# dominikh/jello

Hardware: AMD Instinct MI355X
Metric: Mpixels/sec fine-raster + paths/sec, 100k-path 4096^2 scene (higher is better)
Workload: dtype f32

## Files before the change

### jello_amd/csrc/kernels_tile.hip

```cpp
#include <algorithm>

#include "kcommon.h"

using namespace jk;
using namespace jd;

namespace {

struct Bb4 { float v[4]; };

JD void bbox_intersect(const float* a, const float* b, float* o) {
    float r0 = fmax_(a[0], b[0]), r1 = fmax_(a[1], b[1]), r2 = fmin_(a[2], b[2]), r3 = fmin_(a[3], b[3]);
    o[0] = r0; o[1] = r1; o[2] = r2; o[3] = r3;
}

template <int PASS>
__global__ __launch_bounds__(JL_WG) void k_binning(const JlConfig* __restrict__ cfg, Buf<JlDrawMonoid> draw_monoids, Buf<JlPathBbox> path_bbox_buf,
                                                   Buf<Bb4> clip_bbox_buf, Buf<Bb4> intersected_bbox, JlBump* __restrict__ bump,
                                                   Buf<uint32_t> bin_data, Buf<JlBinHeader> bin_header, uint32_t* __restrict__ wg_tot) {
    __shared__ uint32_t sh_bitmaps[8][JL_N_TILE];
    __shared__ uint32_t sh[8];
    const float SX = 0.00390625f, SY = 0.00390625f;
    uint32_t lid = threadIdx.x;
    uint32_t gid = blockIdx.x * JL_WG + lid;
// ... 139 lines not shown
    const MonoidK<2> sums = block_reduce_monoid<2>(part, sh);
    __syncthreads();
    const uint32_t wg_off = sums.v[0], total = sums.v[1];
    if (blockIdx.x >= write_blocks) {
        tile_zero_part(cfg, total, tiles, blockIdx.x - write_blocks, gridDim.x - write_blocks);
        return;
    }
    if (blockIdx.x == 0u && threadIdx.x == 0u) bump->tile = total;
    uint32_t wg_first = blockIdx.x * JL_WG;
    uint32_t drawobj_ix = wg_first + threadIdx.x;
    uint32_t wg_cnt;
    uint32_t my_sub = block_excl_scan_u32(counts[drawobj_ix], sh, &wg_cnt);
    uint32_t offset = wg_off;
    if (offset + wg_cnt > cfg->tiles_size) {
        offset = 0u;
        if (threadIdx.x == JL_WG - 1u) atomicOr(&bump->failed, (uint32_t)JL_STAGE_TILE_ALLOC);
    }
    if (drawobj_ix < cfg->layout.n_drawobj && paths.ok(drawobj_ix)) paths.p[drawobj_ix].tiles = offset + my_sub;
}
JD void tile_zero_part(const JlConfig* __restrict__ cfg, uint32_t total, Buf<JlTile> tiles, uint32_t block, uint32_t blocks) {
    const uint32_t n = umin_(umin_(total, cfg->tiles_size), tiles.n);
    uint4* p = (uint4*)tiles.p;
    const uint32_t n2 = n >> 1;
    for (uint32_t i = block * JL_WG + threadIdx.x; i < n2; i += blocks * JL_WG) p[i] = make_uint4(0u, 0u, 0u, 0u);
    if ((n & 1u) != 0u && block == 0u && threadIdx.x == 0u) {
        JlTile z;
        z.backdrop = 0;
        z.segment_count_or_ix = 0u;
        tiles.p[n - 1u] = z;
    }
}

__global__ void k_path_count_setup(const JlBump* __restrict__ bump, JlIndirectCount* __restrict__ ind) {
    if (bump->failed != 0u) ind->x = 0u; else ind->x = (bump->lines + (JL_WG - 1u)) / JL_WG;
    ind->y = 1u;
    ind->z = 1u;
}
__global__ void k_path_tiling_setup(const JlBump* __restrict__ bump, JlIndirectCount* __restrict__ ind, Buf<uint32_t> ptcl) {
    if (bump->failed != 0u) {
        ind->x = 0u;
        ptcl.wr(0u, ~0u);
    } else {
        ind->x = (bump->seg_counts + (JL_WG - 1u)) / JL_WG;
    }
    ind->y = 1u;
    ind->z = 1u;
}

#define ONE_MINUS_ULP 0.99999994f
#define ROBUST_EPSILON 2e-7f
#define TILE_SCALE 0.0625f

struct LineSetup {
    bool valid;
    bool is_down, is_positive_slope;
    float a, b, x0, y0, x_sign, s0y;
    uint32_t imin, imax;
    int32_t ymin, ymax, delta;
    int32_t bbox[4];
    int32_t stride;
    uint32_t tiles;
};

JD LineSetup line_setup(const JlLineSoup& line, const Buf<JlPath>& paths) {
    LineSetup r;
    r.valid = false;
    V2 lp0 = v2(line.p0[0], line.p0[1]), lp1 = v2(line.p1[0], line.p1[1]);
    bool is_down = lp1.y >= lp0.y;
    V2 xy0 = is_down ? lp0 : lp1;
    V2 xy1 = is_down ? lp1 : lp0;
    V2 s0 = xy0 * TILE_SCALE;
    V2 s1 = xy1 * TILE_SCALE;
    uint32_t count_x = cell_span(s0.x, s1.x) - 1u;
    uint32_t count = count_x + cell_span(s0.y, s1.y);
    float dx = abs_(s1.x - s0.x);
    float dy = s1.y - s0.y;
    if (dx + dy == 0.0f) return r;
    if (dy == 0.0f && floor_(s0.y) == s0.y) return r;
    float idxdy = 1.0f / (dx + dy);
    float a = dx * idxdy;
    bool is_positive_slope = s1.x >= s0.x;
    float x_sign = is_positive_slope ? 1.0f : -1.0f;
    float xt0 = floor_(s0.x * x_sign);
    float c = s0.x * x_sign - xt0;
    float y0 = floor_(s0.y);
    float ytop = (s0.y == s1.y) ? ceil_(s0.y) : (y0 + 1.0f);
    float b = fmin_((dy * c + dx * (ytop - s0.y)) * idxdy, ONE_MINUS_ULP);
    float robust_err = floor_(a * ((float)count - 1.0f) + b) - (float)count_x;
    if (robust_err != 0.0f) a -= ROBUST_EPSILON * sign_(robust_err);
    float x0 = xt0 * x_sign + (is_positive_slope ? 0.0f : -1.0f);

    JlPath path = paths.rd(line.path_ix);
    int32_t bbox[4] = {(int32_t)path.bbox[0], (int32_t)path.bbox[1], (int32_t)path.bbox[2], (int32_t)path.bbox[3]};
    float xmin = fmin_(s0.x, s1.x);
    int32_t stride = bbox[2] - bbox[0];
    if (s0.y >= (float)bbox[3] || s1.y <= (float)bbox[1] || xmin >= (float)bbox[2] || stride == 0) return r;
    uint32_t imin = 0u;
    if (s0.y < (float)bbox[1]) {
        float iminf = round_(((float)bbox[1] - y0 + b - a) / (1.0f - a)) - 1.0f;
        if (y0 + iminf - floor_(a * iminf + b) < (float)bbox[1]) iminf += 1.0f;
        imin = to_u32(iminf);
    }
    uint32_t imax = count;
    if (s1.y > (float)bbox[3]) {
        float imaxf = round_(((float)bbox[3] - y0 + b - a) / (1.0f - a)) - 1.0f;
        if (y0 + imaxf - floor_(a * imaxf + b) < (float)bbox[3]) imaxf += 1.0f;
        imax = to_u32(imaxf);
    }
    int32_t delta = is_down ? -1 : 1;
    int32_t ymin = 0, ymax = 0;
    if (fmax_(s0.x, s1.x) <= (float)bbox[0]) {
        ymin = to_i32(ceil_(s0.y));
        ymax = to_i32(ceil_(s1.y));
        imax = imin;
    } else {
        float fudge = is_positive_slope ? 0.0f : 1.0f;
        if (xmin < (float)bbox[0]) {
            float f = round_((x_sign * ((float)bbox[0] - x0) - b + fudge) / a);
            if ((x0 + x_sign * floor_(a * f + b) < (float)bbox[0]) == is_positive_slope) f += 1.0f;
            int32_t ynext = to_i32(y0 + f - floor_(a * f + b) + 1.0f);
            if (is_positive_slope) {
                if (to_u32(f) > imin) {
                    ymin = to_i32(y0 + ((y0 == s0.y) ? 0.0f : 1.0f));
                    ymax = ynext;
                    imin = to_u32(f);
                }
            } else {
                if (to_u32(f) < imax) {
                    ymin = ynext;
                    ymax = to_i32(ceil_(s1.y));
                    imax = to_u32(f);
                }
            }
        }
        if (fmax_(s0.x, s1.x) > (float)bbox[2]) {
            float f = round_((x_sign * ((float)bbox[2] - x0) - b + fudge) / a);
            if ((x0 + x_sign * floor_(a * f + b) < (float)bbox[2]) == is_positive_slope) f += 1.0f;
            if (is_positive_slope) imax = umin_(imax, to_u32(f)); else imin = umax_(imin, to_u32(f));
        }
    }
    imax = umax_(imin, imax);
    ymin = imax_(ymin, bbox[1]);
    ymax = imin_(ymax, bbox[3]);
    r.valid = true;
    r.is_down = is_down; r.is_positive_slope = is_positive_slope;
    r.a = a; r.b = b; r.x0 = x0; r.y0 = y0; r.x_sign = x_sign; r.s0y = s0.y;
    r.imin = imin; r.imax = imax; r.ymin = ymin; r.ymax = ymax; r.delta = delta;
    r.bbox[0] = bbox[0]; r.bbox[1] = bbox[1]; r.bbox[2] = bbox[2]; r.bbox[3] = bbox[3];
    r.stride = stride;
    r.tiles = path.tiles;
    return r;
}

__global__ __launch_bounds__(JL_WG) void k_pc_count(const JlBump* __restrict__ bump, const JlIndirectCount* __restrict__ ind, Buf<JlLineSoup> lines,
                                                    Buf<JlPath> paths, uint32_t* __restrict__ counts, uint32_t counts_n,
                                                    uint32_t* __restrict__ zero, uint32_t zero_n, uint32_t* __restrict__ ptotal, uint32_t ptotal_n,
                                                    unsigned long long* __restrict__ bd_ctr,
                                                    JlIndirectCount* __restrict__ setup_out) {
    for (uint32_t i = blockIdx.x * JL_WG + threadIdx.x; i < zero_n; i += gridDim.x * JL_WG) zero[i] = 0u;
    if (blockIdx.x == 0u && threadIdx.x == 0u) *bd_ctr = 0ull;
    uint32_t n_lines = umin_(bump->lines, counts_n);
    uint32_t ind_x;
    if (setup_out) {
        ind_x = bump->failed != 0u ? 0u : (bump->lines + (JL_WG - 1u)) / JL_WG;
        if (blockIdx.x == 0u && threadIdx.x == 0u) { setup_out->x = ind_x; setup_out->y = 1u; setup_out->z = 1u; }
    } else {
        ind_x = ind->x;
    }
    uint32_t n_threads = umin_(ind_x * JL_WG, counts_n);
    const uint32_t lane = lane_id();
    for (uint32_t g0 = blockIdx.x * JL_WG + (threadIdx.x & ~63u); g0 < n_lines; g0 += gridDim.x * JL_WG) {
        const uint32_t gid = g0 + lane;
        uint32_t c = 0u, pix = 0xffffffffu;
        if (gid < n_lines && gid < n_threads && lines.ok(gid)) {
            pix = lines.p[gid].path_ix;
            LineSetup s = line_setup(lines.p[gid], paths);
            if (s.valid) c = s.imax - s.imin;
        }
        if (gid < n_lines) counts[gid] = c;
        const uint32_t incl = wave_incl_scan_u32(c);
        const uint32_t prev = lane_prev(pix, ~pix);
        const uint64_t heads = __builtin_amdgcn_ballot_w64(lane == 0u || pix != prev);
        const uint32_t leader = 63u - (uint32_t)__builtin_clzll(heads & ((2ull << lane) - 1ull));
        const uint32_t lead_incl = (uint32_t)__shfl((int)incl, (int)leader, 64), lead_c = (uint32_t)__shfl((int)c, (int)leader, 64);
        const bool last_of_run = lane == 63u || ((heads >> (lane + 1u)) & 1ull) != 0ull;
        const uint32_t run_sum = incl - (lead_incl - lead_c);
        if (last_of_run && run_sum != 0u && pix < ptotal_n) atomicAdd(&ptotal[pix], run_sum);
    }
}
JD void path_range(uint32_t P, const uint32_t* __restrict__ pstart, const uint32_t* __restrict__ pend, const uint32_t*, const uint32_t*,
                   uint32_t& ps, uint32_t& pe) {
    ps = pstart[P];
    pe = pend[P];
}

#ifndef PC_BIG_PATH
#define PC_BIG_PATH 64u
#endif
JD bool npe_big(uint32_t n) { return n > PC_BIG_PATH; }

#define PC_LONG_LINE 32u
struct EmitCtx {
    const JlConfig* cfg;
    const JlBump* bump;
    Buf<JlTile> tile;
    Buf<JlSegmentCount> seg_counts;
    uint2* tile_of;
    uint32_t* keys;
    uint32_t* kbig;
    uint32_t tile_of_n;
};
JD bool pc_key_is_big(uint32_t key) { return key != 0xffffffffu && (key >> 31) != 0u; }
JD void emit_backdrop_row(const EmitCtx& c, const LineSetup& s, int32_t y) {
    uint32_t base = (uint32_t)((int32_t)s.tiles + (y - s.bbox[1]) * s.stride);
    if (c.tile.ok(base)) atomicAdd(&c.tile.p[base].backdrop, s.delta);
}
template <bool DEFER>
JD void emit_crossing(const EmitCtx& c, const LineSetup& s, uint32_t i, uint32_t gid, uint32_t seg_base, bool big, uint32_t& want_t,
                      uint32_t& want_ix) {
    want_t = 0u;
    want_ix = 0xffffffffu;
    float last_z = floor_(s.a * ((float)i - 1.0f) + s.b);
    float zf = s.a * (float)i + s.b;
    float z = floor_(zf);
    int32_t y = to_i32(s.y0 + (float)i - z);
    int32_t x = to_i32(s.x0 + s.x_sign * z);
    int32_t base = (int32_t)s.tiles + (y - s.bbox[1]) * s.stride - s.bbox[0];
    bool top_edge = (i == 0u) ? (s.y0 == s.s0y) : (last_z == z);
    if (top_edge && x + 1 < s.bbox[2]) {
        int32_t x_bump = imax_(x + 1, s.bbox[0]);
        uint32_t t = (uint32_t)(base + x_bump);
        if (c.tile.ok(t)) atomicAdd(&c.tile.p[t].backdrop, s.delta);
    }
    uint32_t t = (uint32_t)(base + x);
    uint32_t seg_ix = seg_base + i - s.imin;
    if (seg_ix < c.cfg->seg_counts_size && c.seg_counts.ok(seg_ix)) {
        JlSegmentCount sc;
        sc.line_ix = gid;
        sc.counts = i;
        c.seg_counts.p[seg_ix] = sc;
        if (seg_ix < c.tile_of_n) {
            c.keys[seg_ix] = c.tile.ok(t) ? (t | (big ? 0x80000000u : 0u)) : 0xffffffffu;
            if (big) {
                if (DEFER) {
                    want_t = t;
                    want_ix = seg_ix;
                } else {
                    uint32_t arrival = 0u;
                    if (c.tile.ok(t)) arrival = atomicAdd(&c.tile.p[t].segment_count_or_ix, 1u);
                    c.tile_of[seg_ix] = make_uint2(t, arrival);
                }
            }
        }
    }
}

__global__ __launch_bounds__(JL_WG) void k_pc_emit(const JlConfig* __restrict__ cfg, const JlBump* __restrict__ bump,
                                                   const JlIndirectCount* __restrict__ ind, Buf<JlLineSoup> lines, Buf<JlPath> paths, Buf<JlTile> tile,
                                                   Buf<JlSegmentCount> seg_counts, const uint32_t* __restrict__ seg_bases, uint32_t bases_n,
                                                   uint2* __restrict__ tile_of, uint32_t* __restrict__ keys, uint32_t* __restrict__ kbig,
                                                   uint32_t tile_of_n, uint32_t* __restrict__ pfirst, uint32_t* __restrict__ plast,
                                                   const uint32_t* __restrict__ ptotal, uint32_t n_paths, uint32_t* __restrict__ gate) {
    EmitCtx c;
    c.cfg = cfg; c.bump = bump; c.tile = tile; c.seg_counts = seg_counts; c.tile_of = tile_of; c.keys = keys; c.kbig = kbig;
    c.tile_of_n = tile_of_n;
    const uint32_t n_lines = umin_(umin_(bump->lines, bases_n), ind->x * JL_WG);
    const uint32_t lane = lane_id();
    for (uint32_t g0 = blockIdx.x * JL_WG + (threadIdx.x & ~63u); g0 < n_lines; g0 += gridDim.x * JL_WG) {
        const uint32_t gid = g0 + lane;
        LineSetup s;
        s.valid = false;
        uint32_t P = 0xffffffffu;
        uint32_t edgeP = 0xffffffffu;
        if (lane == 0u && gid > 0u && gid - 1u < n_lines && lines.ok(gid - 1u)) edgeP = lines.p[gid - 1u].path_ix;
        if (lane == 63u && gid + 1u < n_lines && lines.ok(gid + 1u)) edgeP = lines.p[gid + 1u].path_ix;
        if (gid < n_lines && lines.ok(gid)) {
            P = lines.p[gid].path_ix;
            s = line_setup(lines.p[gid], paths);
        }
        bool big = true;
        uint32_t seg_base = 0u;
        if (gid < n_lines) seg_base = seg_bases[gid];
        if (s.valid) {
            if (P < n_paths) big = ptotal[P] > PC_BIG_PATH;
        } else {
            s.imin = 0u; s.imax = 0u; s.ymin = 0; s.ymax = 0;
        }
        {
            uint32_t prevP = lane_prev(P, 0u), nextP = lane_next(P, 0u);
            if (lane == 0u) prevP = edgeP;
            if (lane == 63u) nextP = edgeP;
            if (gid < n_lines && P < n_paths) {
                if (P != prevP) pfirst[P] = seg_base;
                if (P != nextP) plast[P] = seg_base + (s.valid ? s.imax - s.imin : 0u);
            }
        }
        if (__builtin_amdgcn_ballot_w64(s.valid && big && s.imax > s.imin) != 0ull && lane == 0u) {
            const uint32_t want = bump->tile;
            if (__hip_atomic_load(gate, __ATOMIC_RELAXED, __HIP_MEMORY_SCOPE_AGENT) < want) atomicMax(gate, want);
        }
        const bool is_long = s.valid && (s.imax - s.imin > PC_LONG_LINE || s.ymax - s.ymin > (int32_t)PC_LONG_LINE);
        const bool per_lane = s.valid && !is_long;
        if (per_lane)
            for (int32_t y = s.ymin; y < s.ymax; y++) emit_backdrop_row(c, s, y);
        uint32_t dummy_t, dummy_ix;
        if (__builtin_amdgcn_ballot_w64(per_lane && big) == 0ull) {
            if (per_lane)
                for (uint32_t i = s.imin; i < s.imax; i++) emit_crossing<false>(c, s, i, gid, seg_base, big, dummy_t, dummy_ix);
        } else {
            const uint32_t trip = per_lane ? s.imax - s.imin : 0u;
            const uint32_t max_trip = (uint32_t)__builtin_amdgcn_readlane((int)wave_incl_max_u32(trip), 63);
            for (uint32_t r = 0u; r < max_trip; r++) {
                uint32_t t = 0u, ix = 0xffffffffu;
                if (r < trip) emit_crossing<true>(c, s, s.imin + r, gid, seg_base, big, t, ix);
                const bool want = ix != 0xffffffffu && c.tile.ok(t);
                const uint32_t key = want ? t : 0xffffffffu - lane;
                const uint32_t prev = (uint32_t)__shfl_up((int)key, 1, 64);
                const bool head = lane == 0u || key != prev;
                const uint64_t heads = __builtin_amdgcn_ballot_w64(head);
                const uint32_t leader = 63u - (uint32_t)__builtin_clzll(heads & ((2ull << lane) - 1ull));
                const uint64_t later = leader == 63u ? 0ull : heads >> (leader + 1u);
                const uint32_t run = later == 0ull ? 64u - leader : (uint32_t)__builtin_ctzll(later) + 1u;
                uint32_t first = 0u;
                if (want && lane == leader) first = atomicAdd(&c.tile.p[t].segment_count_or_ix, run);
                first = (uint32_t)__shfl((int)first, (int)leader, 64);
                if (ix != 0xffffffffu) c.tile_of[ix] = make_uint2(t, want ? first + (lane - leader) : 0u);
            }
        }
        uint64_t m = __builtin_amdgcn_ballot_w64(is_long);
        while (m != 0ull) {
            const uint32_t src = (uint32_t)__builtin_ctzll(m);
            m &= m - 1ull;
            LineSetup t;
            t.valid = true; t.is_down = false; t.is_positive_slope = false;
            t.a = read_lane(s.a, src); t.b = read_lane(s.b, src); t.x0 = read_lane(s.x0, src); t.y0 = read_lane(s.y0, src);
            t.x_sign = read_lane(s.x_sign, src); t.s0y = read_lane(s.s0y, src);
            t.imin = read_lane(s.imin, src); t.imax = read_lane(s.imax, src);
            t.ymin = read_lane(s.ymin, src); t.ymax = read_lane(s.ymax, src); t.delta = read_lane(s.delta, src);
            t.bbox[0] = read_lane(s.bbox[0], src); t.bbox[1] = read_lane(s.bbox[1], src); t.bbox[2] = read_lane(s.bbox[2], src); t.bbox[3] = read_lane(s.bbox[3], src);
            t.stride = read_lane(s.stride, src); t.tiles = read_lane(s.tiles, src);
            const uint32_t t_gid = g0 + src, t_seg_base = read_lane(seg_base, src);
            const bool t_big = read_lane(big ? 1u : 0u, src) != 0u;
            for (int32_t y = t.ymin + (int32_t)lane; y < t.ymax; y += 64) emit_backdrop_row(c, t, y);
            for (uint32_t i = t.imin + lane; i < t.imax; i += 64u) emit_crossing<false>(c, t, i, t_gid, t_seg_base, t_big, dummy_t, dummy_ix);
        }
    }
}

#ifndef PCR_K
#define PCR_K 16u
#endif
struct PcScatterArgs {
    const uint2* tile_of;
    const uint32_t* list_base;
    uint32_t tiles_cap;
    uint32_t* list;
    const uint32_t* kbig;
    uint32_t* gate;
    uint32_t* dense;
    uint32_t dense_cap, blocks;
};
JD void pc_scatter_part(const JlConfig* __restrict__ cfg, const JlBump* __restrict__ bump, Buf<JlTile> tile,
                        const uint2* __restrict__ tile_of, uint32_t n_cap, const uint32_t* __restrict__ list_base,
                        uint32_t tiles_cap, uint32_t* __restrict__ list, const uint32_t* __restrict__ kbig,
                        uint32_t* __restrict__ gate, uint32_t* __restrict__ dense, uint32_t dense_cap, uint32_t block, uint32_t blocks);
__global__ __launch_bounds__(JL_WG) void k_pc_rank_small(const JlConfig* __restrict__ cfg, const JlBump* __restrict__ bump, Buf<JlTile> tile,
                                                         const uint32_t* __restrict__ keys, uint32_t n_cap, const uint32_t* __restrict__ pfirst,
                                                         const uint32_t* __restrict__ plast, const uint32_t* __restrict__ counts,
                                                         const uint32_t* __restrict__ seg_bases, uint32_t n_paths,
                                                         Buf<JlSegmentCount> seg_counts, PcScatterArgs sc, uint32_t* __restrict__ ptotal_zero,
                                                         uint32_t ptotal_words) {
    for (uint32_t i = blockIdx.x * JL_WG + threadIdx.x; i < ptotal_words; i += gridDim.x * JL_WG) ptotal_zero[i] = 0u;
    const uint32_t rank_blocks = gridDim.x - sc.blocks;
    if (blockIdx.x >= rank_blocks) {
        pc_scatter_part(cfg, bump, tile, sc.tile_of, n_cap, sc.list_base, sc.tiles_cap, sc.list, sc.kbig, sc.gate, sc.dense, sc.dense_cap,
                        blockIdx.x - rank_blocks, sc.blocks);
        return;
    }
    const uint32_t n = umin_(umin_(bump->seg_counts, cfg->seg_counts_size), n_cap);
    const uint32_t lane = lane_id();
    const uint32_t waves = (rank_blocks * JL_WG) >> 6;
    const uint32_t wave_ix = (blockIdx.x * JL_WG + threadIdx.x) >> 6;
    const uint32_t n_tasks = (n_paths + PCR_K - 1u) / PCR_K;
    auto load_ranges = [&](uint32_t task, uint32_t& ps, uint32_t& pe) {
        ps = 0u; pe = 0u;
        const uint32_t P = task * PCR_K + lane;
        if (task < n_tasks && lane < PCR_K && P < n_paths) path_range(P, pfirst, plast, counts, seg_bases, ps, pe);
    };
    uint32_t t_ps = 0u, t_pe = 0u;
    uint64_t todo = 0ull;
    uint32_t task = wave_ix;
    uint32_t r_ps, r_pe;
    load_ranges(task, r_ps, r_pe);
    bool task_loaded = false;
    auto advance = [&](uint32_t& cs, uint32_t& ce) -> bool {
        for (;;) {
            if (todo != 0ull) {
                const uint32_t a = (uint32_t)__builtin_ctzll(todo);
                todo &= todo - 1ull;
                cs = (uint32_t)__builtin_amdgcn_readlane((int)t_ps, (int)a);
                ce = (uint32_t)__builtin_amdgcn_readlane((int)t_pe, (int)a);
                while (todo != 0ull) {
                    const uint32_t b2 = (uint32_t)__builtin_ctzll(todo);
                    const uint32_t nps = (uint32_t)__builtin_amdgcn_readlane((int)t_ps, (int)b2);
                    const uint32_t npe = (uint32_t)__builtin_amdgcn_readlane((int)t_pe, (int)b2);
                    if (nps != ce || npe - cs > 64u) break;
                    ce = npe;
                    todo &= todo - 1ull;
                }
                return true;
            }
            if (task_loaded) task += waves;
            if (task >= n_tasks) return false;
            task_loaded = true;
            const uint32_t ps = r_ps, pe_all = r_pe;
            load_ranges(task + waves, r_ps, r_pe);
            t_ps = ps;
            t_pe = umin_(pe_all, n);
            todo = __builtin_amdgcn_ballot_w64(lane < PCR_K && t_pe > ps && !npe_big(pe_all - ps));
        }
    };
    auto fetch = [&](uint32_t cs, uint32_t ce, uint32_t& key, uint32_t& cw) {
        key = 0xffffffffu; cw = 0u;
        const uint32_t k = cs + lane;
        if (k < ce) {
            key = keys[k];
            if (seg_counts.ok(k)) cw = seg_counts.p[k].counts;
        }
    };
    uint32_t c_s = 0u, c_e = 0u, key1 = 0xffffffffu, cw1 = 0u;
    bool have = advance(c_s, c_e);
    if (have) fetch(c_s, c_e, key1, cw1);
    while (have) {
        const uint32_t cs = c_s, ce = c_e;
        const uint32_t my_key = key1, my_cw = cw1;
        have = advance(c_s, c_e);
        if (have) fetch(c_s, c_e, key1, cw1);
        const uint32_t k = cs + lane;
        const bool valid = k < ce;
        const uint32_t my_t = valid ? my_key : 0xffffffffu;
        const bool mine = valid && my_t != 0xffffffffu;
        uint32_t before = 0u, after = 0u;
        uint64_t rem = __builtin_amdgcn_ballot_w64(mine);
        uint32_t grp_lo = 0u, grp_hi = 0u;
        while (rem != 0ull) {
            const uint32_t t = (uint32_t)__builtin_amdgcn_readlane((int)my_t, (int)__builtin_ctzll(rem));
            const bool eq = my_t == t;
            const uint64_t m = __builtin_amdgcn_ballot_w64(eq);
            grp_lo = eq ? (uint32_t)m : grp_lo;
            grp_hi = eq ? (uint32_t)(m >> 32) : grp_hi;
            rem &= ~m;
        }
        if (mine) {
            before = __builtin_amdgcn_mbcnt_hi(grp_hi, __builtin_amdgcn_mbcnt_lo(grp_lo, 0u));
            after = (uint32_t)__builtin_popcount(grp_lo) + (uint32_t)__builtin_popcount(grp_hi) - 1u - before;
        }
        if (mine && seg_counts.ok(k)) {
            seg_counts.p[k].counts = my_cw | (before << 16);
            if (after == 0u && tile.ok(my_t)) tile.p[my_t].segment_count_or_ix = before + 1u;
        }
    }
}

#define PC_DENSE_TILE 16u
#define PC_DENSE_LDS 1024u
JD void pc_scatter_part(const JlConfig* __restrict__ cfg, const JlBump* __restrict__ bump, Buf<JlTile> tile,
                        const uint2* __restrict__ tile_of, uint32_t n_cap, const uint32_t* __restrict__ list_base,
                        uint32_t tiles_cap, uint32_t* __restrict__ list, const uint32_t* __restrict__ kbig,
                        uint32_t* __restrict__ gate, uint32_t* __restrict__ dense, uint32_t dense_cap, uint32_t block, uint32_t blocks) {
    if (*gate == 0u) return;
    uint32_t n = umin_(umin_(bump->seg_counts, cfg->seg_counts_size), n_cap);
    const uint32_t lane = lane_id();
    for (uint32_t k0 = block * JL_WG + (threadIdx.x & ~63u); k0 < n; k0 += blocks * JL_WG) {
        const uint32_t k = k0 + lane;
        bool first_of_dense = false;
        uint32_t t = 0u;
        if (k < n && pc_key_is_big(kbig[k])) {
            uint2 ta = tile_of[k];
            if (ta.x < tiles_cap && tile.ok(ta.x)) {
                uint32_t pos = list_base[ta.x] + ta.y;
                if (pos < n_cap) list[pos] = k;
                t = ta.x;
                first_of_dense = ta.y == 0u && tile.p[t].segment_count_or_ix > PC_DENSE_TILE;
            }
        }
        const uint64_t m = __builtin_amdgcn_ballot_w64(first_of_dense);
        if (m != 0ull) {
            uint32_t at = 0u;
            if (lane == 0u) at = atomicAdd(&gate[1], (uint32_t)__builtin_popcountll(m));
            at = uni(at) + __builtin_amdgcn_mbcnt_hi((uint32_t)(m >> 32), __builtin_amdgcn_mbcnt_lo((uint32_t)m, 0u));
            if (first_of_dense && at < dense_cap) dense[at] = t;
        }
    }
}
__global__ __launch_bounds__(JL_WG) void k_pc_rank(const JlConfig* __restrict__ cfg, const JlBump* __restrict__ bump, Buf<JlTile> tile,
                                                   const uint2* __restrict__ tile_of, uint32_t n_cap, const uint32_t* __restrict__ list_base,
                                                   uint32_t tiles_cap, const uint32_t* __restrict__ list, Buf<JlSegmentCount> seg_counts,
                                                   const uint32_t* __restrict__ kbig, const uint32_t* __restrict__ gate,
                                                   const uint32_t* __restrict__ dense, uint32_t dense_cap) {
    __shared__ uint32_t sh_list[JL_WG / 64][PC_DENSE_LDS];
    if (*gate == 0u) return;
    uint32_t n = umin_(umin_(bump->seg_counts, cfg->seg_counts_size), n_cap);
    for (uint32_t k = blockIdx.x * JL_WG + threadIdx.x; k < n; k += gridDim.x * JL_WG) {
        if (!pc_key_is_big(kbig[k])) continue;
        uint32_t t = tile_of[k].x;
        if (t >= tiles_cap || !tile.ok(t) || !seg_counts.ok(k)) continue;
        uint32_t cnt = tile.p[t].segment_count_or_ix;
        if (cnt > PC_DENSE_TILE) continue;
        uint32_t base = list_base[t];
        uint32_t rank = 0u;
        for (uint32_t j = 0; j < cnt; j++) {
            uint32_t pos = base + j;
            if (pos < n_cap && list[pos] < k) rank++;
        }
        seg_counts.p[k].counts |= rank << 16;
    }
    const uint32_t lane = lane_id(), wv = threadIdx.x >> 6;
    uint32_t* my_list = sh_list[wv];
    const uint32_t n_dense = umin_(gate[1], dense_cap);
    const uint32_t waves = (gridDim.x * JL_WG) >> 6;
    for (uint32_t d = uni((blockIdx.x * JL_WG + threadIdx.x) >> 6); d < n_dense; d += waves) {
        const uint32_t t = uni(dense[d]);
        if (t >= tiles_cap || !tile.ok(t)) continue;
        const uint32_t base = uni(list_base[t]);
        uint32_t m = uni(tile.p[t].segment_count_or_ix);
        if (base >= n_cap) continue;
        m = umin_(m, n_cap - base);
        for (uint32_t o0 = 0u; o0 < m; o0 += PC_DENSE_LDS) {
            const uint32_t on = umin_(m - o0, PC_DENSE_LDS);
            wave_sync();
            for (uint32_t i = lane; i < ((on + 3u) & ~3u); i += 64u) my_list[i] = i < on ? list[base + o0 + i] : 0xffffffffu;
            wave_sync();
            for (uint32_t j = lane; j < m; j += 64u) {
                const uint32_t e = list[base + j];
                uint32_t r = 0u;
                for (uint32_t i = 0u; i < on; i += 4u) {
                    const uint4 q = *(const uint4*)&my_list[i];
                    r += (q.x < e ? 1u : 0u) + (q.y < e ? 1u : 0u) + (q.z < e ? 1u : 0u) + (q.w < e ? 1u : 0u);
                }
                if (seg_counts.ok(e)) seg_counts.p[e].counts += r << 16;
// ... 155 lines not shown
        bool is_positive_slope = s1.x >= s0.x;
        float x_sign = is_positive_slope ? 1.0f : -1.0f;
        float xt0 = floor_(s0.x * x_sign);
        float c = s0.x * x_sign - xt0;
        float y0i = floor_(s0.y);
        float ytop = (s0.y == s1.y) ? ceil_(s0.y) : (y0i + 1.0f);
        float b = fmin_((dy * c + dx * (ytop - s0.y)) * idxdy, ONE_MINUS_ULP);
        float robust_err = floor_(a * ((float)count - 1.0f) + b) - (float)count_x;
        if (robust_err != 0.0f) a -= ROBUST_EPSILON * sign_(robust_err);
        int32_t x0i = to_i32(xt0 * x_sign + 0.5f * (x_sign - 1.0f));
        float z = floor_(a * (float)seg_within_line + b);
        int32_t x = x0i + to_i32(x_sign * z);
        int32_t y = to_i32(y0i + (float)seg_within_line - z);
        JlPath path = paths.rd(line.path_ix);
        int32_t bbox[4] = {(int32_t)path.bbox[0], (int32_t)path.bbox[1], (int32_t)path.bbox[2], (int32_t)path.bbox[3]};
        int32_t stride = bbox[2] - bbox[0];
        int32_t tile_ix = (int32_t)path.tiles + (y - bbox[1]) * stride + x - bbox[0];
        JlTile tile = tiles.rd((uint32_t)tile_ix);
        uint32_t seg_start = ~tile.segment_count_or_ix;
        if ((int32_t)seg_start < 0) continue;
        V2 tile_xy = v2((float)x * 16.0f, (float)y * 16.0f);
        V2 tile_xy1 = tile_xy + v2(16.0f, 16.0f);
        if (seg_within_line > 0u) {
            float z_prev = floor_(a * ((float)seg_within_line - 1.0f) + b);
            if (z == z_prev) {
                float xt = xy0.x + (xy1.x - xy0.x) * (tile_xy.y - xy0.y) / (xy1.y - xy0.y);
                xt = clamp_(xt, tile_xy.x + 1e-3f, tile_xy1.x);
                xy0 = v2(xt, tile_xy.y);
            } else {
                float x_clip = is_positive_slope ? tile_xy.x : tile_xy1.x;
                float yt = xy0.y + (xy1.y - xy0.y) * (x_clip - xy0.x) / (xy1.x - xy0.x);
                yt = clamp_(yt, tile_xy.y + 1e-3f, tile_xy1.y);
                xy0 = v2(x_clip, yt);
            }
        }
        if (seg_within_line < count - 1u) {
            float z_next = floor_(a * ((float)seg_within_line + 1.0f) + b);
            if (z == z_next) {
                float xt = xy0.x + (xy1.x - xy0.x) * (tile_xy1.y - xy0.y) / (xy1.y - xy0.y);
                xt = clamp_(xt, tile_xy.x + 1e-3f, tile_xy1.x);
                xy1 = v2(xt, tile_xy1.y);
            } else {
                float x_clip = is_positive_slope ? tile_xy1.x : tile_xy.x;
                float yt = xy0.y + (xy1.y - xy0.y) * (x_clip - xy0.x) / (xy1.x - xy0.x);
                yt = clamp_(yt, tile_xy.y + 1e-3f, tile_xy1.y);
                xy1 = v2(x_clip, yt);
            }
        }
        float y_edge = 1e9f;
        V2 p0 = xy0 - tile_xy;
        V2 p1 = xy1 - tile_xy;
        const float EPSILON = 1e-6f;
        if (p0.x == 0.0f) {
            if (p1.x == 0.0f) {
                p0.x = EPSILON;
                if (p0.y == 0.0f) {
                    p1.x = EPSILON;
                    p1.y = 16.0f;
                } else {
                    p1.x = 2.0f * EPSILON;
                    p1.y = p0.y;
                }
            } else if (p0.y == 0.0f) {
                p0.x = EPSILON;
            } else {
                y_edge = p0.y;
            }
        } else if (p1.x == 0.0f) {
            if (p1.y == 0.0f) p1.x = EPSILON; else y_edge = p1.y;
        }
        if (p0.x == floor_(p0.x) && p0.x != 0.0f) p0.x -= EPSILON;
        if (p1.x == floor_(p1.x) && p1.x != 0.0f) p1.x -= EPSILON;
        if (!is_down) { V2 tmp = p0; p0 = p1; p1 = tmp; }
        JlSegment seg;
        seg.p0[0] = p0.x; seg.p0[1] = p0.y; seg.p1[0] = p1.x; seg.p1[1] = p1.y; seg.y_edge = y_edge; seg.pad = 0u;
        segments.wr(seg_start + seg_within_slice, seg);
    }
}



}

#ifndef TILE_GRID_PER_CU
#define TILE_GRID_PER_CU 8
#endif
#ifndef PC_EMIT_GRID_PER_CU
#define PC_EMIT_GRID_PER_CU 32
#endif
static inline uint32_t stride_grid(const JhLaunch& L, uint64_t n_items, uint32_t per_cu = TILE_GRID_PER_CU) {
    uint64_t blocks = (n_items + JL_WG - 1) / JL_WG;
    uint64_t cap = (uint64_t)L.cus() * per_cu;
    if (blocks > cap) blocks = cap;
    if (blocks == 0) blocks = 1;
    return (uint32_t)blocks;
}

enum { BN_CFG, BN_DRAW_MONOID, BN_PATH_BBOX, BN_CLIP_BBOX, BN_INTERSECTED_BBOX, BN_BUMP, BN_BIN_DATA, BN_BIN_HEADER };
JhResult jh_launch_binning(const JhLaunch& L) {
    if (L.gx == 0) return JH_L_OK;
    uint32_t* wg_tot = (uint32_t*)jh_scratch_get(L.scratch, JH_SCR_A, (uint64_t)L.gx * 4);
    if (!wg_tot) return JH_L_SCRATCH;
    auto cfg = L.ptr<const JlConfig>(BN_CFG);
    auto dm = L.buf<JlDrawMonoid>(BN_DRAW_MONOID);
    auto pb = L.buf<JlPathBbox>(BN_PATH_BBOX);
    auto cb = L.buf<Bb4>(BN_CLIP_BBOX);
    auto ib = L.buf<Bb4>(BN_INTERSECTED_BBOX);
    JlBump* bump = L.ptr<JlBump>(BN_BUMP);
    auto bd = L.buf<uint32_t>(BN_BIN_DATA);
    auto bh = L.buf<JlBinHeader>(BN_BIN_HEADER);
    hipLaunchKernelGGL(k_binning<0>, dim3(L.gx), dim3(JL_WG), 0, L.stream, cfg, dm, pb, cb, ib, bump, bd, bh, wg_tot);
    hipLaunchKernelGGL(k_binning<1>, dim3(L.gx), dim3(JL_WG), 0, L.stream, cfg, dm, pb, cb, ib, bump, bd, bh, wg_tot);
    return JH_L_OK;
}

enum { TA_CFG, TA_SCENE, TA_DRAW_BBOX, TA_BUMP, TA_PATHS, TA_TILES };
JhResult jh_launch_tile_alloc(const JhLaunch& L) {
    if (L.gx == 0) return JH_L_OK;
    uint32_t n = L.gx * JL_WG;
    uint32_t* counts = (uint32_t*)jh_scratch_get(L.scratch, JH_SCR_A, (uint64_t)n * 4);
    uint32_t* wg_tot = (uint32_t*)jh_scratch_get(L.scratch, JH_SCR_B, (uint64_t)L.gx * 4);
    if (!counts || !wg_tot) return JH_L_SCRATCH;
    auto cfg = L.ptr<const JlConfig>(TA_CFG);
    auto scene = L.buf<uint32_t>(TA_SCENE);
    auto db = L.buf<Bb4>(TA_DRAW_BBOX);
    JlBump* bump = L.ptr<JlBump>(TA_BUMP);
    auto paths = L.buf<JlPath>(TA_PATHS);
    auto tiles = L.buf<JlTile>(TA_TILES);
    hipLaunchKernelGGL(k_tile_alloc_count, dim3(L.gx), dim3(JL_WG), 0, L.stream, cfg, scene, db, (const JlBump*)bump, paths, counts, wg_tot);
    hipLaunchKernelGGL(k_tile_alloc_write, dim3(L.gx + stride_grid(L, (uint64_t)tiles.n / 2u + 1u)), dim3(JL_WG), 0, L.stream, cfg, bump, paths, tiles,
                       (const uint32_t*)counts, (const uint32_t*)wg_tot, L.gx);
    return JH_L_OK;
}

JhResult jh_launch_path_count_setup(const JhLaunch& L) {
    hipLaunchKernelGGL(k_path_count_setup, dim3(1), dim3(1), 0, L.stream, L.ptr<const JlBump>(PCS_BUMP), L.ptr<JlIndirectCount>(PCS_INDIRECT));
    return JH_L_OK;
}
JhResult jh_launch_path_tiling_setup(const JhLaunch& L) {
    hipLaunchKernelGGL(k_path_tiling_setup, dim3(1), dim3(1), 0, L.stream, L.ptr<const JlBump>(PTS_BUMP), L.ptr<JlIndirectCount>(PTS_INDIRECT),
                       L.buf<uint32_t>(PTS_PTCL));
    return JH_L_OK;
}

JhResult jh_launch_path_count(const JhLaunch& L) {
    auto cfg = L.ptr<const JlConfig>(PC_CFG);
    JlBump* bump = L.ptr<JlBump>(PC_BUMP);
    auto lines = L.buf<JlLineSoup>(PC_LINES);
    auto paths = L.buf<JlPath>(PC_PATHS);
    auto tile = L.buf<JlTile>(PC_TILES);
    auto segc = L.buf<JlSegmentCount>(PC_SEGC);
    auto ind = (const JlIndirectCount*)L.indirect;
    uint32_t lines_cap = lines.n, seg_cap = segc.n, tiles_cap = tile.n;
    uint32_t* counts = (uint32_t*)jh_scratch_get(L.scratch, JH_SCR_A, (uint64_t)lines_cap * 4);
    uint32_t* bases = (uint32_t*)jh_scratch_get(L.scratch, JH_SCR_B, (uint64_t)lines_cap * 4);
    uint2* tile_of = (uint2*)jh_scratch_get(L.scratch, JH_SCR_C, (uint64_t)seg_cap * 8);
    uint32_t* list = (uint32_t*)jh_scratch_get(L.scratch, JH_SCR_D, (uint64_t)seg_cap * 4);
    uint32_t* list_base = (uint32_t*)jh_scratch_get(L.scratch, JH_SCR_E, (uint64_t)tiles_cap * 4);
    uint32_t* keys = (uint32_t*)jh_scratch_get(L.scratch, JH_SCR_F, (uint64_t)seg_cap * 4);
    uint32_t* kbig = keys;
    uint32_t n_paths = paths.n;
    const uint32_t dense_cap = seg_cap / PC_DENSE_TILE + 1u;
    uint32_t* dense = (uint32_t*)jh_scratch_get(L.scratch, JH_SCR_G, (uint64_t)dense_cap * 4);
    if (!dense) return JH_L_SCRATCH;
    uint32_t* prange = (uint32_t*)jh_scratch_get(L.scratch, JH_SCR_I, ((uint64_t)n_paths * 3 + 64) * 4);
    if (!counts || !bases || !tile_of || !list || !list_base || !keys || !kbig || !prange) return JH_L_SCRATCH;
    uint32_t *pfirst = prange, *plast = prange + n_paths, *gate = prange + 2 * (size_t)n_paths;
    uint32_t gl = stride_grid(L, lines_cap), gs = stride_grid(L, seg_cap);
    unsigned long long* bd_ctr = (unsigned long long*)jh_scratch_get(L.scratch, JH_SCR_BD_CTR, 64);
    if (!bd_ctr) return JH_L_SCRATCH;
    uint32_t* ptotal = (uint32_t*)jh_scratch_acquire(L.scratch, JH_SCR_PC_TOT, (uint64_t)n_paths * 4, 0xffffffffull * 4, L.stream);
    if (!ptotal) return JH_L_SCRATCH;
    const uint32_t ptotal_words = (uint32_t)std::min<uint64_t>(jh_scratch_cap(L.scratch, JH_SCR_PC_TOT) / 4, 0xffffffffull);
    hipLaunchKernelGGL(k_pc_count, dim3(gl), dim3(JL_WG), 0, L.stream, (const JlBump*)bump, ind, lines, paths, counts, lines_cap, prange,
                       n_paths * 2u + 64u, ptotal, n_paths, bd_ctr, L.absorbed.write_indirect ? (JlIndirectCount*)L.indirect : (JlIndirectCount*)nullptr);
    jh_scratch_left_clean(L.scratch, JH_SCR_BD_CTR);
    JhResult rc = jh_scan_u32(L, counts, 1, bases, lines_cap, &bump->lines, &bump->seg_counts);
    if (rc) return rc;
    const uint32_t *cpf = pfirst, *cpl = plast, *cc = counts, *cb = bases;
    hipLaunchKernelGGL(k_pc_emit, dim3(stride_grid(L, lines_cap, PC_EMIT_GRID_PER_CU)), dim3(JL_WG), 0, L.stream, cfg, (const JlBump*)bump, ind, lines, paths, tile, segc, cb, lines_cap,
                       tile_of, keys, kbig, seg_cap, pfirst, plast, (const uint32_t*)ptotal, n_paths, gate);
    rc = jh_scan_u32(L, ((const uint32_t*)tile.p) + 1, 2, list_base, tiles_cap, gate, nullptr);
    if (rc) return rc;
    PcScatterArgs sc;
    sc.tile_of = tile_of; sc.list_base = list_base; sc.tiles_cap = tiles_cap; sc.list = list; sc.kbig = kbig; sc.gate = gate; sc.dense = dense;
    sc.dense_cap = dense_cap; sc.blocks = gs;
    hipLaunchKernelGGL(k_pc_rank_small, dim3(gs + stride_grid(L, (uint64_t)n_paths * 64u)), dim3(JL_WG), 0, L.stream, cfg, (const JlBump*)bump, tile,
                       (const uint32_t*)keys, seg_cap, cpf, cpl, cc, cb, n_paths, segc, sc, ptotal, ptotal_words);
    jh_scratch_left_clean(L.scratch, JH_SCR_PC_TOT);
    hipLaunchKernelGGL(k_pc_rank, dim3(gs), dim3(JL_WG), 0, L.stream, cfg, (const JlBump*)bump, tile, (const uint2*)tile_of, seg_cap,
                       (const uint32_t*)list_base, tiles_cap, (const uint32_t*)list, segc, (const uint32_t*)kbig, (const uint32_t*)gate,
                       (const uint32_t*)dense, dense_cap);
    return JH_L_OK;
}

enum { BD_CFG, BD_BUMP, BD_PATHS, BD_TILES };
JhResult jh_launch_backdrop_dyn(const JhLaunch& L) {
    if (L.gx == 0) return JH_L_OK;
    auto paths = L.buf<JlPath>(BD_PATHS);
    auto tiles = L.buf<JlTile>(BD_TILES);
    const uint32_t wide_cap = paths.n;
    uint8_t* w = (uint8_t*)jh_scratch_get(L.scratch, JH_SCR_A, 64 + (uint64_t)wide_cap * sizeof(uint4));
    if (!w) return JH_L_SCRATCH;
    unsigned long long* wide_ctr = (unsigned long long*)jh_scratch_acquire(L.scratch, JH_SCR_BD_CTR, 64, 8, L.stream);
    if (!wide_ctr) return JH_L_SCRATCH;
    uint4* wide_list = (uint4*)(w + 64);
    const uint32_t wide_min = L.gx < 64u ? 2u : BD_WIDE;
    hipLaunchKernelGGL(k_backdrop_dyn, dim3(L.gx), dim3(JL_WG), 0, L.stream, L.ptr<const JlConfig>(BD_CFG), L.ptr<const JlBump>(BD_BUMP), paths, tiles,
                       wide_ctr, wide_list, wide_cap, wide_min);
    hipLaunchKernelGGL(k_backdrop_wide, dim3(stride_grid(L, (uint64_t)wide_cap * 64u * 64u)), dim3(JL_WG), 0, L.stream, L.ptr<const JlBump>(BD_BUMP), tiles,
                       (const unsigned long long*)wide_ctr, (const uint4*)wide_list, wide_cap);
    return JH_L_OK;
}

JhResult jh_launch_path_tiling(const JhLaunch& L) {
    auto segc = L.buf<JlSegmentCount>(PT_SEGC);
    uint32_t g = stride_grid(L, segc.n);
    const JhBound& ptcl = L.absorbed.tiling_ptcl;
    hipLaunchKernelGGL(k_path_tiling, dim3(g), dim3(JL_WG), 0, L.stream, L.ptr<const JlBump>(PT_BUMP), (const JlIndirectCount*)L.indirect, segc,
                       L.buf<JlLineSoup>(PT_LINES), L.buf<JlPath>(PT_PATHS), L.buf<JlTile>(PT_TILES), L.buf<JlSegment>(PT_SEGMENTS),
                       L.absorbed.write_indirect ? (JlIndirectCount*)L.indirect : (JlIndirectCount*)nullptr, mkbuf<uint32_t>(ptcl.ptr, ptcl.size));
    return JH_L_OK;
}
```

Baseline: 20990.

## Scan per-wave segment sums instead of per-line counts in path-coarse

k_pc_count now writes one inclusive sum per 64-line wave instead of a count per line, and the device scan runs over wave sums, which is 64x shorter. k_pc_emit recomputes line_setup counts and rebuilds per-line segment bases with an in-wave scan added to the wave base. This removes the per-line counts/bases buffers and most of the scan's memory traffic. In exchange, emit does the count and wave scan again, and the scan length now depends on a device-written wave count.

```diff
diff --git a/jello_amd/csrc/kernels_tile.hip b/jello_amd/csrc/kernels_tile.hip
--- a/jello_amd/csrc/kernels_tile.hip
+++ b/jello_amd/csrc/kernels_tile.hip
@@ -315,14 +315,27 @@
     return r;
 }
 
+JD uint32_t pc_line_limit(const JlBump* __restrict__ bump, uint32_t ind_x, uint32_t lines_cap) {
+    return umin_(umin_(bump->lines, lines_cap), ind_x * JL_WG);
+}
+JD uint32_t pc_waves(uint32_t n_lines) { return (n_lines >> 6) + ((n_lines & 63u) != 0u ? 1u : 0u); }
+JD uint32_t pc_line_count(const Buf<JlLineSoup>& lines, const Buf<JlPath>& paths, uint32_t gid, uint32_t n_lines, LineSetup& s, uint32_t& pix) {
+    s.valid = false;
+    pix = 0xffffffffu;
+    if (gid < n_lines && lines.ok(gid)) {
+        pix = lines.p[gid].path_ix;
+        s = line_setup(lines.p[gid], paths);
+    }
+    return s.valid ? s.imax - s.imin : 0u;
+}
+
 __global__ __launch_bounds__(JL_WG) void k_pc_count(const JlBump* __restrict__ bump, const JlIndirectCount* __restrict__ ind, Buf<JlLineSoup> lines,
-                                                    Buf<JlPath> paths, uint32_t* __restrict__ counts, uint32_t counts_n,
+                                                    Buf<JlPath> paths, uint32_t* __restrict__ wsum, uint32_t lines_cap, uint32_t* __restrict__ n_waves_out,
                                                     uint32_t* __restrict__ zero, uint32_t zero_n, uint32_t* __restrict__ ptotal, uint32_t ptotal_n,
                                                     unsigned long long* __restrict__ bd_ctr,
                                                     JlIndirectCount* __restrict__ setup_out) {
     for (uint32_t i = blockIdx.x * JL_WG + threadIdx.x; i < zero_n; i += gridDim.x * JL_WG) zero[i] = 0u;
     if (blockIdx.x == 0u && threadIdx.x == 0u) *bd_ctr = 0ull;
-    uint32_t n_lines = umin_(bump->lines, counts_n);
     uint32_t ind_x;
     if (setup_out) {
         ind_x = bump->failed != 0u ? 0u : (bump->lines + (JL_WG - 1u)) / JL_WG;
@@ -330,18 +343,16 @@
     } else {
         ind_x = ind->x;
     }
-    uint32_t n_threads = umin_(ind_x * JL_WG, counts_n);
+    const uint32_t n_lines = pc_line_limit(bump, ind_x, lines_cap);
+    if (blockIdx.x == 0u && threadIdx.x == 0u) *n_waves_out = pc_waves(n_lines);
     const uint32_t lane = lane_id();
     for (uint32_t g0 = blockIdx.x * JL_WG + (threadIdx.x & ~63u); g0 < n_lines; g0 += gridDim.x * JL_WG) {
         const uint32_t gid = g0 + lane;
-        uint32_t c = 0u, pix = 0xffffffffu;
-        if (gid < n_lines && gid < n_threads && lines.ok(gid)) {
-            pix = lines.p[gid].path_ix;
-            LineSetup s = line_setup(lines.p[gid], paths);
-            if (s.valid) c = s.imax - s.imin;
-        }
-        if (gid < n_lines) counts[gid] = c;
+        LineSetup s;
+        uint32_t pix;
+        const uint32_t c = pc_line_count(lines, paths, gid, n_lines, s, pix);
         const uint32_t incl = wave_incl_scan_u32(c);
+        if (lane == 63u) wsum[g0 >> 6] = incl;
         const uint32_t prev = lane_prev(pix, ~pix);
         const uint64_t heads = __builtin_amdgcn_ballot_w64(lane == 0u || pix != prev);
         const uint32_t leader = 63u - (uint32_t)__builtin_clzll(heads & ((2ull << lane) - 1ull));
@@ -351,8 +362,7 @@
         if (last_of_run && run_sum != 0u && pix < ptotal_n) atomicAdd(&ptotal[pix], run_sum);
     }
 }
-JD void path_range(uint32_t P, const uint32_t* __restrict__ pstart, const uint32_t* __restrict__ pend, const uint32_t*, const uint32_t*,
-                   uint32_t& ps, uint32_t& pe) {
+JD void path_range(uint32_t P, const uint32_t* __restrict__ pstart, const uint32_t* __restrict__ pend, uint32_t& ps, uint32_t& pe) {
     ps = pstart[P];
     pe = pend[P];
 }
@@ -420,30 +430,26 @@
 
 __global__ __launch_bounds__(JL_WG) void k_pc_emit(const JlConfig* __restrict__ cfg, const JlBump* __restrict__ bump,
                                                    const JlIndirectCount* __restrict__ ind, Buf<JlLineSoup> lines, Buf<JlPath> paths, Buf<JlTile> tile,
-                                                   Buf<JlSegmentCount> seg_counts, const uint32_t* __restrict__ seg_bases, uint32_t bases_n,
+                                                   Buf<JlSegmentCount> seg_counts, const uint32_t* __restrict__ wbase, uint32_t lines_cap,
                                                    uint2* __restrict__ tile_of, uint32_t* __restrict__ keys, uint32_t* __restrict__ kbig,
                                                    uint32_t tile_of_n, uint32_t* __restrict__ pfirst, uint32_t* __restrict__ plast,
                                                    const uint32_t* __restrict__ ptotal, uint32_t n_paths, uint32_t* __restrict__ gate) {
     EmitCtx c;
     c.cfg = cfg; c.bump = bump; c.tile = tile; c.seg_counts = seg_counts; c.tile_of = tile_of; c.keys = keys; c.kbig = kbig;
     c.tile_of_n = tile_of_n;
-    const uint32_t n_lines = umin_(umin_(bump->lines, bases_n), ind->x * JL_WG);
+    const uint32_t n_lines = pc_line_limit(bump, ind->x, lines_cap);
     const uint32_t lane = lane_id();
     for (uint32_t g0 = blockIdx.x * JL_WG + (threadIdx.x & ~63u); g0 < n_lines; g0 += gridDim.x * JL_WG) {
         const uint32_t gid = g0 + lane;
-        LineSetup s;
-        s.valid = false;
-        uint32_t P = 0xffffffffu;
+        const uint32_t wave_base = wbase[g0 >> 6];
         uint32_t edgeP = 0xffffffffu;
         if (lane == 0u && gid > 0u && gid - 1u < n_lines && lines.ok(gid - 1u)) edgeP = lines.p[gid - 1u].path_ix;
         if (lane == 63u && gid + 1u < n_lines && lines.ok(gid + 1u)) edgeP = lines.p[gid + 1u].path_ix;
-        if (gid < n_lines && lines.ok(gid)) {
-            P = lines.p[gid].path_ix;
-            s = line_setup(lines.p[gid], paths);
-        }
+        LineSetup s;
+        uint32_t P;
+        const uint32_t cnt = pc_line_count(lines, paths, gid, n_lines, s, P);
+        const uint32_t seg_base = wave_base + (wave_incl_scan_u32(cnt) - cnt);
         bool big = true;
-        uint32_t seg_base = 0u;
-        if (gid < n_lines) seg_base = seg_bases[gid];
         if (s.valid) {
             if (P < n_paths) big = ptotal[P] > PC_BIG_PATH;
         } else {
@@ -455,7 +461,7 @@
             if (lane == 63u) nextP = edgeP;
             if (gid < n_lines && P < n_paths) {
                 if (P != prevP) pfirst[P] = seg_base;
-                if (P != nextP) plast[P] = seg_base + (s.valid ? s.imax - s.imin : 0u);
+                if (P != nextP) plast[P] = seg_base + cnt;
             }
         }
         if (__builtin_amdgcn_ballot_w64(s.valid && big && s.imax > s.imin) != 0ull && lane == 0u) {
@@ -529,8 +535,7 @@
                         uint32_t* __restrict__ gate, uint32_t* __restrict__ dense, uint32_t dense_cap, uint32_t block, uint32_t blocks);
 __global__ __launch_bounds__(JL_WG) void k_pc_rank_small(const JlConfig* __restrict__ cfg, const JlBump* __restrict__ bump, Buf<JlTile> tile,
                                                          const uint32_t* __restrict__ keys, uint32_t n_cap, const uint32_t* __restrict__ pfirst,
-                                                         const uint32_t* __restrict__ plast, const uint32_t* __restrict__ counts,
-                                                         const uint32_t* __restrict__ seg_bases, uint32_t n_paths,
+                                                         const uint32_t* __restrict__ plast, uint32_t n_paths,
                                                          Buf<JlSegmentCount> seg_counts, PcScatterArgs sc, uint32_t* __restrict__ ptotal_zero,
                                                          uint32_t ptotal_words) {
     for (uint32_t i = blockIdx.x * JL_WG + threadIdx.x; i < ptotal_words; i += gridDim.x * JL_WG) ptotal_zero[i] = 0u;
@@ -548,7 +553,7 @@
     auto load_ranges = [&](uint32_t task, uint32_t& ps, uint32_t& pe) {
         ps = 0u; pe = 0u;
         const uint32_t P = task * PCR_K + lane;
-        if (task < n_tasks && lane < PCR_K && P < n_paths) path_range(P, pfirst, plast, counts, seg_bases, ps, pe);
+        if (task < n_tasks && lane < PCR_K && P < n_paths) path_range(P, pfirst, plast, ps, pe);
     };
     uint32_t t_ps = 0u, t_pe = 0u;
     uint64_t todo = 0ull;
@@ -1010,8 +1015,9 @@
     auto segc = L.buf<JlSegmentCount>(PC_SEGC);
     auto ind = (const JlIndirectCount*)L.indirect;
     uint32_t lines_cap = lines.n, seg_cap = segc.n, tiles_cap = tile.n;
-    uint32_t* counts = (uint32_t*)jh_scratch_get(L.scratch, JH_SCR_A, (uint64_t)lines_cap * 4);
-    uint32_t* bases = (uint32_t*)jh_scratch_get(L.scratch, JH_SCR_B, (uint64_t)lines_cap * 4);
+    const uint32_t waves_cap = (uint32_t)(((uint64_t)lines_cap + 63u) / 64u), waves_pad = (waves_cap + 15u) & ~15u;
+    uint32_t* wsum = (uint32_t*)jh_scratch_get(L.scratch, JH_SCR_A, ((uint64_t)waves_pad + 16u) * 4);
+    uint32_t* wbase = (uint32_t*)jh_scratch_get(L.scratch, JH_SCR_B, (uint64_t)waves_pad * 4);
     uint2* tile_of = (uint2*)jh_scratch_get(L.scratch, JH_SCR_C, (uint64_t)seg_cap * 8);
     uint32_t* list = (uint32_t*)jh_scratch_get(L.scratch, JH_SCR_D, (uint64_t)seg_cap * 4);
     uint32_t* list_base = (uint32_t*)jh_scratch_get(L.scratch, JH_SCR_E, (uint64_t)tiles_cap * 4);
@@ -1022,7 +1028,8 @@
     uint32_t* dense = (uint32_t*)jh_scratch_get(L.scratch, JH_SCR_G, (uint64_t)dense_cap * 4);
     if (!dense) return JH_L_SCRATCH;
     uint32_t* prange = (uint32_t*)jh_scratch_get(L.scratch, JH_SCR_I, ((uint64_t)n_paths * 3 + 64) * 4);
-    if (!counts || !bases || !tile_of || !list || !list_base || !keys || !kbig || !prange) return JH_L_SCRATCH;
+    if (!wsum || !wbase || !tile_of || !list || !list_base || !keys || !kbig || !prange) return JH_L_SCRATCH;
+    uint32_t* n_waves_dev = wsum + waves_pad;
     uint32_t *pfirst = prange, *plast = prange + n_paths, *gate = prange + 2 * (size_t)n_paths;
     uint32_t gl = stride_grid(L, lines_cap), gs = stride_grid(L, seg_cap);
     unsigned long long* bd_ctr = (unsigned long long*)jh_scratch_get(L.scratch, JH_SCR_BD_CTR, 64);
@@ -1030,12 +1037,12 @@
     uint32_t* ptotal = (uint32_t*)jh_scratch_acquire(L.scratch, JH_SCR_PC_TOT, (uint64_t)n_paths * 4, 0xffffffffull * 4, L.stream);
     if (!ptotal) return JH_L_SCRATCH;
     const uint32_t ptotal_words = (uint32_t)std::min<uint64_t>(jh_scratch_cap(L.scratch, JH_SCR_PC_TOT) / 4, 0xffffffffull);
-    hipLaunchKernelGGL(k_pc_count, dim3(gl), dim3(JL_WG), 0, L.stream, (const JlBump*)bump, ind, lines, paths, counts, lines_cap, prange,
+    hipLaunchKernelGGL(k_pc_count, dim3(gl), dim3(JL_WG), 0, L.stream, (const JlBump*)bump, ind, lines, paths, wsum, lines_cap, n_waves_dev, prange,
                        n_paths * 2u + 64u, ptotal, n_paths, bd_ctr, L.absorbed.write_indirect ? (JlIndirectCount*)L.indirect : (JlIndirectCount*)nullptr);
     jh_scratch_left_clean(L.scratch, JH_SCR_BD_CTR);
-    JhResult rc = jh_scan_u32(L, counts, 1, bases, lines_cap, &bump->lines, &bump->seg_counts);
+    JhResult rc = jh_scan_u32(L, wsum, 1, wbase, waves_cap, n_waves_dev, &bump->seg_counts);
     if (rc) return rc;
-    const uint32_t *cpf = pfirst, *cpl = plast, *cc = counts, *cb = bases;
+    const uint32_t *cpf = pfirst, *cpl = plast, *cb = wbase;
     hipLaunchKernelGGL(k_pc_emit, dim3(stride_grid(L, lines_cap, PC_EMIT_GRID_PER_CU)), dim3(JL_WG), 0, L.stream, cfg, (const JlBump*)bump, ind, lines, paths, tile, segc, cb, lines_cap,
                        tile_of, keys, kbig, seg_cap, pfirst, plast, (const uint32_t*)ptotal, n_paths, gate);
     rc = jh_scan_u32(L, ((const uint32_t*)tile.p) + 1, 2, list_base, tiles_cap, gate, nullptr);
@@ -1044,7 +1051,7 @@
     sc.tile_of = tile_of; sc.list_base = list_base; sc.tiles_cap = tiles_cap; sc.list = list; sc.kbig = kbig; sc.gate = gate; sc.dense = dense;
     sc.dense_cap = dense_cap; sc.blocks = gs;
     hipLaunchKernelGGL(k_pc_rank_small, dim3(gs + stride_grid(L, (uint64_t)n_paths * 64u)), dim3(JL_WG), 0, L.stream, cfg, (const JlBump*)bump, tile,
-                       (const uint32_t*)keys, seg_cap, cpf, cpl, cc, cb, n_paths, segc, sc, ptotal, ptotal_words);
+                       (const uint32_t*)keys, seg_cap, cpf, cpl, n_paths, segc, sc, ptotal, ptotal_words);
     jh_scratch_left_clean(L.scratch, JH_SCR_PC_TOT);
     hipLaunchKernelGGL(k_pc_rank, dim3(gs), dim3(JL_WG), 0, L.stream, cfg, (const JlBump*)bump, tile, (const uint2*)tile_of, seg_cap,
                        (const uint32_t*)list_base, tiles_cap, (const uint32_t*)list, segc, (const uint32_t*)kbig, (const uint32_t*)gate,
```

Result: faster. 21630 (median of 6 runs) (+3.0%).
